# vt-asaplab/vPIN

Measured on AMD Instinct MI355X. Metric: R1CS constraints/sec, whole Spartan SNARK (sat proof + SPARK evaluation proof; vPIN point-mult + point-add instances), higher is better.
Workload: dtype u256 (integers mod q and mod p = 2^255-19, 32-bit limbs); 1 GPU; vPIN LeNet trace (layers L1..L7): 12 SNARKs per step; inputs=resident in HBM, parallelism=one trace per rank x 1 rank(s), no collective; 4 stream(s) per rank, table_slot_bytes=128

## Files before the change

vpin_amd/csrc/msm.hip:

```cpp
#include <algorithm>
#include <atomic>
#include <cstdlib>
#include <condition_variable>
#include <cstring>
#include <memory>
#include <mutex>
#include <string>
#include <vector>

#include "ctx.h"
#include "fp_dev.h"
#include "fp10_dev.h"
#include "ge_tree_dev.h"
#include "mailbox_dev.h"

#ifndef VPIN_NIELS_SLOT
#define VPIN_NIELS_SLOT 96
#endif
static_assert(VPIN_NIELS_SLOT == 96 || VPIN_NIELS_SLOT == 128, "table entry size");

struct vpin_gens {
  vpin::fp* table = nullptr;
  vpin::fp* table_hi = nullptr;
  int s32 = VPIN_NIELS_SLOT / 32;
// ... 217 lines not shown
  int off = w * c, word = off >> 5, sh = off & 31;
  uint32_t lo = s.v[word], hi = (word + 1 < 8) ? s.v[word + 1] : 0u;
  uint64_t both = ((uint64_t)hi << 32) | lo;
  return (uint32_t)(both >> sh) & ((1u << c) - 1u);
}

__device__ __forceinline__ uint32_t carry_into(const fq& s, int w0, int c) {
  const uint32_t half = 1u << (c - 1);
  for (int w = w0 - 1; w >= 0; w--) {
    uint32_t d = scalar_digit(s, w, c);
    if (d != half) return d > half ? 1u : 0u;
  }
  return 0u;
}

__device__ __forceinline__ void table_mul_acc_range(ge_ext& acc, const fq& s_in, const TableSeg& sg, int w0, int w1) {
  fq s = s_in;
  const bool flip = fq_fold_sign(s);
  uint32_t carry = carry_into(s, w0, sg.c);
  const uint32_t full = 1u << sg.c, half = 1u << (sg.c - 1);
#pragma unroll 1
  for (int w = w0; w < w1; w++) {
    uint32_t v = scalar_digit(s, w, sg.c) + carry;
    bool neg = v > half;
    uint32_t mag = neg ? full - v : v;
    carry = neg ? 1u : 0u;
    if (mag != 0) acc = ge_add_niels(acc, niels_load(sg.entry(w, mag - 1)), neg != flip);
  }
}


constexpr int kMsmBlock = 256;
constexpr unsigned kSharedPad = 40000u;
constexpr int kSeg = 8192;

template <bool TEN>
__global__ __launch_bounds__(kMsmBlock, 3) void msm_rows_kernel(const fq* __restrict__ Z, size_t stride, size_t ncols,
                                                             const fq* __restrict__ extra, int n_extra, size_t extra_base0,
                                                             TableView tv, ge_ext* __restrict__ out) {
  const size_t row = blockIdx.x;
  RowAcc<TEN> acc;
  const size_t total = ncols + (size_t)n_extra;
  if (ncols >= 256 && (ncols & (ncols - 1)) == 0 && ((size_t)1 << (tv.nbt - tv.sum0 - 1)) >= ncols) {
    const fq* zr = Z + row * stride;
    const fq first = fq_load(zr);
    if (fq_same(first, fq_load(zr + 1)) && fq_same(first, fq_load(zr + ncols / 2)) && fq_same(first, fq_load(zr + ncols - 1))) {
      int same = 1;
      for (size_t j = threadIdx.x; j < ncols; j += kMsmBlock) same &= fq_same(first, fq_load(zr + j)) ? 1 : 0;
      if (__syncthreads_and(same)) {
        if (threadIdx.x == 0) {
          if (blockIdx.y == 0) {
            if (!fq_is_zero(first)) acc.mul_acc(fq_from_mont(first), tv, tv.sum0 + (size_t)(63 - __builtin_clzll((unsigned long long)ncols)));
            for (int e = 0; e < n_extra; e++) {
              const fq x = fq_load(extra + row * (size_t)n_extra + e);
              if (!fq_is_zero(x)) acc.mul_acc(fq_from_mont(x), tv, extra_base0 + e);
            }
          }
          ge_ext* o = out + row * gridDim.y + blockIdx.y;
          const ge_ext av = acc.ext();
          fp_store(&o->X, av.X); fp_store(&o->Y, av.Y); fp_store(&o->Z, av.Z); fp_store(&o->T, av.T);
        }
        return;
      }
    }
  }
  const size_t per = (total + gridDim.y - 1) / gridDim.y;
  const size_t j0 = (size_t)blockIdx.y * per, j1 = (j0 + per < total) ? j0 + per : total;
  __shared__ uint16_t nz_list[kSeg];
  __shared__ uint32_t nz_count;
  for (size_t seg = j0; seg < j1; seg += kSeg) {
    const size_t seg_end = (seg + kSeg < j1) ? seg + kSeg : j1;
    if (threadIdx.x == 0) nz_count = 0;
    __syncthreads();
    for (size_t j = seg + threadIdx.x; j < seg_end; j += kMsmBlock) {
      const fq* sp = (j < ncols) ? (Z + row * stride + j) : (extra + row * (size_t)n_extra + (j - ncols));
      if (!fq_is_zero(fq_load(sp))) nz_list[atomicAdd(&nz_count, 1u)] = (uint16_t)(j - seg);
    }
    __syncthreads();
    const uint32_t cnt = nz_count;
    for (uint32_t k = threadIdx.x; k < cnt; k += kMsmBlock) {
      const size_t j = seg + nz_list[k];
      fq s;
      size_t base;
      if (j < ncols) { s = fq_load(Z + row * stride + j); base = j; }
      else { s = fq_load(extra + row * (size_t)n_extra + (j - ncols)); base = extra_base0 + (j - ncols); }
      acc.mul_acc(fq_from_mont(s), tv, base);
    }
    __syncthreads();
  }
  __shared__ ge_ext sh[kMsmBlock];
  sh[threadIdx.x] = acc.ext();
  __syncthreads();
  ge_tree_quad(sh, kMsmBlock);
  if (threadIdx.x == 0) {
    const ge_ext av = sh[0];
    ge_ext* o = out + row * gridDim.y + blockIdx.y;
    fp_store(&o->X, av.X); fp_store(&o->Y, av.Y); fp_store(&o->Z, av.Z); fp_store(&o->T, av.T);
  }
}

struct HotRows {
  const uint32_t* idx[3];
  uint32_t hot[3];
  const ge_cached* T[3];
  size_t row0, rows_per_vec;
};

__global__ __launch_bounds__(64) void scalar_times_bases_kernel(const fq* __restrict__ vp, size_t n, TableView tv,
                                                                ge_cached* __restrict__ T) {
  const size_t j = (size_t)blockIdx.x * 64 + threadIdx.x;
  if (j >= n) return;
  const fq v = fq_load(vp);
  ge_ext acc = ge_identity();
  if (!fq_is_zero(v)) table_mul_acc(acc, fq_from_mont(v), tv, j);
  const ge_cached cch = ge_to_cached(acc);
  fp_store(&T[j].YpX, cch.YpX); fp_store(&T[j].YmX, cch.YmX); fp_store(&T[j].Z, cch.Z); fp_store(&T[j].T2d, cch.T2d);
}

template <bool TEN>
__global__ __launch_bounds__(kMsmBlock, 3) void msm_rows_hot_kernel(const fq* __restrict__ Z, size_t stride, size_t ncols, TableView tv,
                                                                 HotRows hr, ge_ext* __restrict__ out, size_t row_base, size_t row_step,
                                                                 int z_compact, const uint8_t* __restrict__ strip_flag) {
  const size_t row = row_base + (size_t)blockIdx.x * row_step;
  const fq* zr = Z + (z_compact ? (size_t)blockIdx.x : row) * stride;
  RowAcc<TEN> acc;
  const bool hot_only = strip_flag && strip_flag[blockIdx.x];
  if (!hot_only && ncols >= 256 && (ncols & (ncols - 1)) == 0 && ((size_t)1 << (tv.nbt - tv.sum0 - 1)) >= ncols) {
    const fq first = fq_load(zr);
    if (fq_same(first, fq_load(zr + 1)) && fq_same(first, fq_load(zr + ncols / 2)) && fq_same(first, fq_load(zr + ncols - 1))) {
      int same = 1;
      for (size_t j = threadIdx.x; j < ncols; j += kMsmBlock) same &= fq_same(first, fq_load(zr + j)) ? 1 : 0;
      if (__syncthreads_and(same)) {
        if (threadIdx.x == 0) {
          if (blockIdx.y == 0 && !fq_is_zero(first)) acc.mul_acc(fq_from_mont(first), tv, tv.sum0 + (size_t)(63 - __builtin_clzll((unsigned long long)ncols)));
          ge_ext* o = out + (size_t)blockIdx.x * gridDim.y + blockIdx.y;
          const ge_ext av = acc.ext();
          fp_store(&o->X, av.X); fp_store(&o->Y, av.Y); fp_store(&o->Z, av.Z); fp_store(&o->T, av.T);
        }
        return;
      }
    }
  }
  const uint32_t* idx = nullptr;
  const ge_cached* T = nullptr;
  uint32_t hot = 0xffffffffu;
  if (row >= hr.row0 && row < hr.row0 + 3 * hr.rows_per_vec) {
    const size_t m = (row - hr.row0) / hr.rows_per_vec;
    if (hr.hot[m] != 0xffffffffu) {
      hot = hr.hot[m];
      T = hr.T[m];
      idx = hr.idx[m] + (row - hr.row0 - m * hr.rows_per_vec) * ncols;
    }
  }
  __shared__ uint16_t list[kSeg];
  __shared__ uint32_t n_front, n_back;
  const size_t per = (ncols + gridDim.y - 1) / gridDim.y;
  const size_t c0 = (size_t)blockIdx.y * per, c1 = (c0 + per < ncols) ? c0 + per : ncols;
  for (size_t seg = c0; seg < c1; seg += kSeg) {
    const size_t seg_end = (seg + kSeg < c1) ? seg + kSeg : c1;
    if (threadIdx.x == 0) { n_front = 0; n_back = 0; }
    __syncthreads();
    for (size_t j = seg + threadIdx.x; j < seg_end; j += kMsmBlock) {
      if (fq_is_zero(fq_load(zr + j))) continue;
      if (idx && idx[j] == hot) list[kSeg - 1 - atomicAdd(&n_back, 1u)] = (uint16_t)(j - seg);
      else if (!hot_only) list[atomicAdd(&n_front, 1u)] = (uint16_t)(j - seg);
    }
    __syncthreads();
    const uint32_t nf = n_front, nb = n_back;
    for (uint32_t k = threadIdx.x; k < nf; k += kMsmBlock) {
      const size_t j = seg + list[k];
      acc.mul_acc(fq_from_mont(fq_load(zr + j)), tv, j);
    }
    for (uint32_t k = threadIdx.x; k < nb; k += kMsmBlock) {
      const ge_cached* t = T + seg + list[kSeg - 1 - k];
      ge_cached q;
      q.YpX = fp_load(&t->YpX); q.YmX = fp_load(&t->YmX); q.Z = fp_load(&t->Z); q.T2d = fp_load(&t->T2d);
      acc.add_cached(q);
    }
    __syncthreads();
  }
  __shared__ ge_ext sh[kMsmBlock];
  sh[threadIdx.x] = acc.ext();
  __syncthreads();
  ge_tree_quad(sh, kMsmBlock);
  if (threadIdx.x == 0) {
    const ge_ext av = sh[0];
    ge_ext* o = out + (size_t)blockIdx.x * gridDim.y + blockIdx.y;
    fp_store(&o->X, av.X); fp_store(&o->Y, av.Y); fp_store(&o->Z, av.Z); fp_store(&o->T, av.T);
  }
}



__global__ __launch_bounds__(kMsmBlock) void strip_classify_kernel(const fq* __restrict__ Z, size_t stride, size_t ncols, HotRows hr,
                                                                    size_t row_base, size_t row_step, int z_compact,
                                                                    uint8_t* __restrict__ flag) {
  const size_t row = row_base + (size_t)blockIdx.x * row_step;
  const fq* zr = Z + (z_compact ? (size_t)blockIdx.x : row) * stride;
  const uint32_t* idx = nullptr;
  uint32_t hot = 0xffffffffu;
  if (hr.rows_per_vec && row >= hr.row0 && row < hr.row0 + 3 * hr.rows_per_vec) {
    const size_t m = (row - hr.row0) / hr.rows_per_vec;
    if (hr.hot[m] != 0xffffffffu) { hot = hr.hot[m]; idx = hr.idx[m] + (row - hr.row0 - m * hr.rows_per_vec) * ncols; }
  }
  const fq first = fq_load(zr);
  int same = 1;
  uint32_t skipped = 0;
  for (size_t j = threadIdx.x; j < ncols; j += kMsmBlock) {
    const fq v = fq_load(zr + j);
    same &= fq_same(first, v) ? 1 : 0;
    skipped += (fq_is_zero(v) || (idx && idx[j] == hot)) ? 1u : 0u;
  }
  __shared__ uint32_t sh[kMsmBlock];
  sh[threadIdx.x] = skipped;
  const int all_same = __syncthreads_and(same);
  for (int st = kMsmBlock / 2; st >= 1; st >>= 1) {
    if ((int)threadIdx.x < st) sh[threadIdx.x] += sh[threadIdx.x + st];
    __syncthreads();
  }
  if (threadIdx.x == 0) flag[blockIdx.x] = (!all_same && sh[0] * 8 <= ncols) ? 1 : 0;
}

__global__ __launch_bounds__(1024) void strip_list_kernel(const uint8_t* __restrict__ flag, size_t nrows, uint32_t* __restrict__ list,
                                                           uint32_t* __restrict__ count) {
  __shared__ uint32_t base[1024];
  const size_t per = (nrows + 1023) / 1024, r0 = (size_t)threadIdx.x * per, r1 = r0 + per < nrows ? r0 + per : nrows;
  uint32_t n = 0;
  for (size_t r = r0; r < r1; r++) n += flag[r] ? 1u : 0u;
  base[threadIdx.x] = n;
  __syncthreads();
  if (threadIdx.x == 0) {
    uint32_t run = 0;
    for (int t = 0; t < 1024; t++) { const uint32_t v = base[t]; base[t] = run; run += v; }
    *count = run;
  }
  __syncthreads();
  uint32_t o = base[threadIdx.x];
  for (size_t r = r0; r < r1; r++)
    if (flag[r]) list[o++] = (uint32_t)r;
}

__global__ __launch_bounds__(256) void strip_trim_kernel(const uint32_t* __restrict__ list, uint32_t* __restrict__ count, uint32_t n_use,
                                                          uint32_t n_all, uint8_t* __restrict__ flag) {
  const uint32_t li = n_use + blockIdx.x * 256 + threadIdx.x;
  if (li < n_all) flag[list[li]] = 0;
  if (blockIdx.x == 0 && threadIdx.x == 0) *count = n_use;
}

__global__ __launch_bounds__(kMsmBlock, 3) void msm_strip_kernel(const fq* __restrict__ Z, size_t stride, size_t ncols, TableView tv, HotRows hr,
                                                                  const uint32_t* __restrict__ list, const uint32_t* __restrict__ list_count,
                                                                  int S, size_t row_base, size_t row_step, int z_compact,
                                                                  ge_ext* __restrict__ parts, uint32_t* __restrict__ sync, int lag) {
  const uint32_t n = *list_count;
  const uint32_t s = blockIdx.x % (uint32_t)S, grp = blockIdx.x / (uint32_t)S;
  if (grp * kMsmBlock >= n) return;
  const uint32_t li = grp * kMsmBlock + threadIdx.x;
  const bool live = li < n;
  const uint32_t i = list[live ? li : n - 1];
  const size_t row = row_base + (size_t)i * row_step;
  const fq* zr = Z + (z_compact ? (size_t)i : row) * stride;
  const uint32_t* idx = nullptr;
  uint32_t hot = 0xffffffffu;
  if (hr.rows_per_vec && row >= hr.row0 && row < hr.row0 + 3 * hr.rows_per_vec) {
    const size_t m = (row - hr.row0) / hr.rows_per_vec;
    if (hr.hot[m] != 0xffffffffu) { hot = hr.hot[m]; idx = hr.idx[m] + (row - hr.row0 - m * hr.rows_per_vec) * ncols; }
  }
  const size_t per = (ncols + (size_t)S - 1) / (size_t)S, j0 = (size_t)s * per, j1 = j0 + per < ncols ? j0 + per : ncols;
  ge10 acc = ge10_identity();
  const uint32_t groups = (n + kMsmBlock - 1) / kMsmBlock;
  uint32_t* my_sync = sync ? sync + (size_t)s * (per + 1) : nullptr;
  __shared__ int sh_nosync;
  if (threadIdx.x == 0) sh_nosync = 0;
  __syncthreads();
  for (size_t j = j0; j < j1; j++) {
    if (my_sync && j - j0 >= (size_t)lag) {
      if (threadIdx.x == 0 && !sh_nosync) {
        long spin = 0;
        while (__hip_atomic_load(my_sync + (j - j0 - (size_t)lag), __ATOMIC_RELAXED, __HIP_MEMORY_SCOPE_AGENT) < groups)
          if (++spin > (1L << 16)) { sh_nosync = 1; break; }
      }
      __syncthreads();
    }
    fq v = fq_load(zr + j);
    const bool act = live && !fq_is_zero(v) && !(idx && idx[j] == hot);
    if (__builtin_amdgcn_ballot_w64(act) != 0) {
      fq sc = fq_from_mont(v);
      if (!act) sc = fq_zero();
      table_mul_acc10(acc, sc, tv, j);
    }
    if (my_sync) {
      __syncthreads();
      if (threadIdx.x == 0) __hip_atomic_fetch_add(my_sync + (j - j0), 1u, __ATOMIC_RELAXED, __HIP_MEMORY_SCOPE_AGENT);
    }
  }
  if (live) {
    const ge_ext av = ge10_to_ext(acc);
    ge_ext* o = parts + (size_t)li * (size_t)S + s;
    fp_store(&o->X, av.X); fp_store(&o->Y, av.Y); fp_store(&o->Z, av.Z); fp_store(&o->T, av.T);
  }
}

__global__ __launch_bounds__(64) void strip_combine_kernel(const ge_ext* __restrict__ parts, const uint32_t* __restrict__ list,
                                                            const uint32_t* __restrict__ list_count, int S, ge_ext* __restrict__ out) {
  const uint32_t li = blockIdx.x * 64 + threadIdx.x;
  if (li >= *list_count) return;
  ge_ext* o = out + list[li];
  ge_ext a;
  a.X = fp_load(&o->X); a.Y = fp_load(&o->Y); a.Z = fp_load(&o->Z); a.T = fp_load(&o->T);
  for (int s = 0; s < S; s++) {
    const ge_ext* p = parts + (size_t)li * (size_t)S + s;
    ge_ext q;
    q.X = fp_load(&p->X); q.Y = fp_load(&p->Y); q.Z = fp_load(&p->Z); q.T = fp_load(&p->T);
    a = ge_add(a, q);
  }
  fp_store(&o->X, a.X); fp_store(&o->Y, a.Y); fp_store(&o->Z, a.Z); fp_store(&o->T, a.T);
}

__device__ __forceinline__ uint32_t count_digits(fq s, const TableView& tv, size_t j) {
  (void)fq_fold_sign(s);
  const TableSeg sg = table_seg(tv, j);
  uint32_t carry = 0, n = 0;
  const uint32_t full = 1u << sg.c, half = 1u << (sg.c - 1);
  for (int w = 0; w < sg.W; w++) {
    uint32_t v = scalar_digit(s, w, sg.c) + carry;
    const bool neg = v > half;
    const uint32_t mag = neg ? full - v : v;
    carry = neg ? 1u : 0u;
    n += mag != 0;
  }
  return n;
}
__global__ __launch_bounds__(kMsmBlock) void msm_count_adds_kernel(const fq* __restrict__ Z, size_t stride, size_t ncols,
                                                                   const fq* __restrict__ extra, int n_extra, size_t extra_base0,
                                                                   TableView tv, unsigned long long* __restrict__ count,
                                                                   HotRows hr = HotRows{}, size_t row_base = 0, size_t row_step = 1,
                                                                   int z_compact = 0) {
  const size_t row = row_base + (size_t)blockIdx.x * row_step;
  const fq* zr = Z + (z_compact ? (size_t)blockIdx.x : row) * stride;
  const uint32_t* hidx = nullptr;
  uint32_t hot = 0xffffffffu;
  if (hr.rows_per_vec && row >= hr.row0 && row < hr.row0 + 3 * hr.rows_per_vec) {
    const size_t m = (row - hr.row0) / hr.rows_per_vec;
    if (hr.hot[m] != 0xffffffffu) { hot = hr.hot[m]; hidx = hr.idx[m] + (row - hr.row0 - m * hr.rows_per_vec) * ncols; }
  }
  uint32_t n = 0;
  bool constant = false;
  if (ncols >= 256 && (ncols & (ncols - 1)) == 0 && ((size_t)1 << (tv.nbt - tv.sum0 - 1)) >= ncols) {
    const fq first = fq_load(zr);
    int same = 1;
    for (size_t j = threadIdx.x; j < ncols; j += kMsmBlock) same &= fq_same(first, fq_load(zr + j)) ? 1 : 0;
    constant = __syncthreads_and(same) != 0;
    if (constant && threadIdx.x == 0 && !fq_is_zero(first))
      n += count_digits(fq_from_mont(first), tv, tv.sum0 + (size_t)(63 - __builtin_clzll((unsigned long long)ncols)));
  }
  if (!constant)
    for (size_t j = threadIdx.x; j < ncols; j += kMsmBlock) {
      const fq s = fq_load(zr + j);
      if (!fq_is_zero(s) && !(hidx && hidx[j] == hot)) n += count_digits(fq_from_mont(s), tv, j);
    }
  for (int e = threadIdx.x; e < n_extra; e += kMsmBlock) {
    const fq x = fq_load(extra + row * (size_t)n_extra + e);
    if (!fq_is_zero(x)) n += count_digits(fq_from_mont(x), tv, extra_base0 + e);
  }
  __shared__ uint32_t sh[kMsmBlock];
  sh[threadIdx.x] = n;
  __syncthreads();
  for (int st = kMsmBlock / 2; st >= 1; st >>= 1) {
    if ((int)threadIdx.x < st) sh[threadIdx.x] += sh[threadIdx.x + st];
    __syncthreads();
  }
  if (threadIdx.x == 0 && sh[0]) atomicAdd(count, (unsigned long long)sh[0]);
}

constexpr int kWideScalars = 32;
template <int Q>
__global__ __launch_bounds__(kMsmBlock) void msm_wide_kernel(const fq* __restrict__ S, size_t ncols, TableView tv,
                                                             fp* __restrict__ parts_xyzt) {
  const size_t row = blockIdx.y;
  const int grp = threadIdx.x & 7;
  ge_ext acc = ge_identity();
#pragma unroll 1
  for (int q = 0; q < Q; q++) {
    const size_t j = ((size_t)blockIdx.x * Q + q) * kWideScalars + (threadIdx.x >> 3);
    if (j < ncols) {
      fq s = fq_load(S + row * ncols + j);
      if (!fq_is_zero(s)) {
        const TableSeg sg = table_seg(tv, j);
        const int wpg = (sg.W + 7) / 8;
        int w0 = grp * wpg, w1 = (w0 + wpg < sg.W) ? w0 + wpg : sg.W;
        if (w0 < w1) table_mul_acc_range(acc, fq_from_mont(s), sg, w0, w1);
      }
    }
  }
  __shared__ ge_ext sh[kMsmBlock];
  sh[threadIdx.x] = acc;
  __syncthreads();
  ge_tree_quad(sh, kMsmBlock);
  if (threadIdx.x == 0) {
    acc = sh[0];
    fp* o = parts_xyzt + 4 * (row * gridDim.x + blockIdx.x);
    fp_store(o, fp_freeze(acc.X)); fp_store(o + 1, fp_freeze(acc.Y)); fp_store(o + 2, fp_freeze(acc.Z)); fp_store(o + 3, fp_freeze(acc.T));
  }
}


struct BulletStep {
  const fq* a_prev; const fq* b_prev;
  fq* a_next; fq* b_next;
  fq* sj;
  size_t n, R;
  int fold, finish, nmsm;
  fq u, u_inv;
  fp* parts;
  uint32_t* up;
  uint32_t seq;
};

__global__ __launch_bounds__(kMsmBlock) void bullet_step_kernel(BulletStep a, TableView tv) {
  const size_t n = a.n;
  const int nip = (int)gridDim.x - a.nmsm;
  if ((int)blockIdx.x < nip) {
    const int ib = (int)blockIdx.x;
    const size_t i = (size_t)ib * kMsmBlock + threadIdx.x;
    fq pl = fq_zero(), pr = fq_zero();
    if (a.finish) {
      if (ib == 0 && threadIdx.x == 0) {
        pl = fq_add(fq_mul(fq_load(a.a_prev), a.u), fq_mul(a.u_inv, fq_load(a.a_prev + 1)));
        pr = fq_add(fq_mul(fq_load(a.b_prev), a.u_inv), fq_mul(a.u, fq_load(a.b_prev + 1)));
      }
    } else if (i < n) {
      fq a0, a1, b0, b1;
      if (a.fold) {
        a0 = fq_add(fq_mul(fq_load(a.a_prev + i), a.u), fq_mul(a.u_inv, fq_load(a.a_prev + 2 * n + i)));
        a1 = fq_add(fq_mul(fq_load(a.a_prev + n + i), a.u), fq_mul(a.u_inv, fq_load(a.a_prev + 3 * n + i)));
        b0 = fq_add(fq_mul(fq_load(a.b_prev + i), a.u_inv), fq_mul(a.u, fq_load(a.b_prev + 2 * n + i)));
        b1 = fq_add(fq_mul(fq_load(a.b_prev + n + i), a.u_inv), fq_mul(a.u, fq_load(a.b_prev + 3 * n + i)));
      } else {
        a0 = fq_load(a.a_prev + i); a1 = fq_load(a.a_prev + n + i);
        b0 = fq_load(a.b_prev + i); b1 = fq_load(a.b_prev + n + i);
      }
      fq_store(a.a_next + i, a0); fq_store(a.a_next + n + i, a1);
      fq_store(a.b_next + i, b0); fq_store(a.b_next + n + i, b1);
      pl = fq_mul(a0, b1);
      pr = fq_mul(a1, b0);
    }
    __shared__ fq shp[kMsmBlock / 64][2];
    const int lane = threadIdx.x & 63, wave = threadIdx.x >> 6;
    pl = fq_wave_sum(pl);
    pr = fq_wave_sum(pr);
    if (lane == 0) { shp[wave][0] = pl; shp[wave][1] = pr; }
    __syncthreads();
    if (threadIdx.x < 2) {
      fq t = shp[0][threadIdx.x];
#pragma unroll
      for (int w = 1; w < kMsmBlock / 64; w++) t = fq_add(t, shp[w][threadIdx.x]);
      publish_scalar(a.up + (2 * (size_t)ib + threadIdx.x) * 12, t, a.seq);
    }
    return;
// ... 468 lines not shown

static int msm_rows_pip(vpin_ctx* c, const vpin_gens* g, const fq* dZ, size_t rows, size_t stride, size_t ncols, const fq* d_extra,
                        int n_extra, size_t extra_base0, int cbits, ge_ext* d_points) {
  DevBuf dgn(c);
  if (dgn.alloc((ncols + 1) * sizeof(ge_niels))) return VPIN_ENOMEM;
  hipLaunchKernelGGL(pip_gens_kernel, dim3((unsigned)((ncols + 1 + 255) / 256)), dim3(256), 0, c->stream, view(g), ncols, extra_base0,
                     n_extra, (ge_niels*)dgn.p);
  return pip_rows(c, (const ge_niels*)dgn.p, dZ, rows, stride, ncols, d_extra, n_extra, cbits, d_points,
                  c->prof_count_adds ? c->d_add_count : nullptr);
}

static int msm_rows(vpin_ctx* c, const vpin_gens* g, const fq* dZ, size_t rows, size_t stride, size_t ncols,
                    const fq* d_extra, int n_extra, size_t extra_base0, ge_ext* d_points) {
  if (const int pm = pip_mode())
    if (n_extra <= 1 && ncols + (size_t)n_extra <= 32768)
      return msm_rows_pip(c, g, dZ, rows, stride, ncols, d_extra, n_extra, extra_base0, pm < 0 ? 0 : pm, d_points);
  double nz_est = (double)rows * ((double)ncols + n_extra);
  size_t total = ncols + (size_t)n_extra;
  int chunks = 1;
  if (rows < 128) {
    size_t want = (total + kMsmBlock - 1) / kMsmBlock * 4;
    chunks = (int)(want < 1 ? 1 : want > 64 ? 64 : want);
  } else if (rows >= 768 && total > (size_t)kSeg) {
    static const int env_chunks = [] { const char* e = getenv("VPIN_MSM_ROW_CHUNKS"); return e ? atoi(e) : 0; }();
    chunks = env_chunks > 0 ? env_chunks : (int)std::min<size_t>(8, (total + kSeg - 1) / kSeg);
  } else if (rows < 768 && total >= 2 * (size_t)kMsmBlock) {
    size_t want = (768 + rows - 1) / rows, most = total / kMsmBlock;
    chunks = (int)(want < most ? want : most);
    if (chunks < 1) chunks = 1;
  }
  DevBuf parts(c);
  ge_ext* dst = d_points;
  if (chunks > 1) {
    if (parts.alloc(rows * (size_t)chunks * sizeof(ge_ext))) return VPIN_ENOMEM;
    dst = (ge_ext*)parts.p;
  }
  if (c->prof_count_adds && c->d_add_count && rows >= 128)
    hipLaunchKernelGGL(msm_count_adds_kernel, dim3((unsigned)rows), dim3(kMsmBlock), 0, c->stream, dZ, stride, ncols, d_extra,
                       n_extra, extra_base0, view(g), c->d_add_count);
  {
    ProfScope ps(c, VPIN_K_MSM, 32.0 * nz_est, rows >= 128 ? VPIN_K_MSM_ROWS : -1);
    static const int env_pad = [] { const char* e = getenv("VPIN_MSM_LDS_PAD"); return e ? atoi(e) : -1; }();
    const unsigned pad = env_pad >= 0 ? (unsigned)env_pad : (c->shared_device ? kSharedPad : 0u);
    if (msm_ten_limbs())
      hipLaunchKernelGGL(msm_rows_kernel<true>, dim3((unsigned)rows, (unsigned)chunks), dim3(kMsmBlock), pad, c->stream, dZ, stride,
                         ncols, d_extra, n_extra, extra_base0, view(g), dst);
    else
      hipLaunchKernelGGL(msm_rows_kernel<false>, dim3((unsigned)rows, (unsigned)chunks), dim3(kMsmBlock), pad, c->stream, dZ, stride,
                         ncols, d_extra, n_extra, extra_base0, view(g), dst);
  }
  if (chunks > 1)
    hipLaunchKernelGGL(ge_sum_chunks_kernel, dim3((unsigned)((rows + 63) / 64)), dim3(64), 0, c->stream, (const ge_ext*)dst,
                       rows, chunks, d_points);
  VPIN_HIP_TRY(hipGetLastError());
  return VPIN_OK;
}

int vpin_hyrax_commit(vpin_ctx* c, const vpin_gens* g, const vpin_table* Z, const uint8_t* blinds, size_t L,
                      size_t blind_base, uint8_t* out_compressed) {
  if (!c || !g || !Z || !Z->d || !blinds || !out_compressed || L == 0) return VPIN_EINVAL;
  if (Z->len % L != 0) return VPIN_ESHAPE;
  size_t R = Z->len / L;
  if (R > g->nb || blind_base >= g->nb) return VPIN_ESHAPE;
  (void)hipSetDevice(c->device);
  DevBuf dbl(c), dpts(c), dout(c);
  if (dbl.alloc(L * 32) || dpts.alloc(L * sizeof(ge_ext)) || dout.alloc(L * 32)) return VPIN_ENOMEM;
  VPIN_HIP_TRY(hipMemcpyAsync(dbl.p, blinds, L * 32, hipMemcpyHostToDevice, c->stream));
  int rc = msm_rows(c, g, Z->d, L, R, R, (const fq*)dbl.p, 1, blind_base, (ge_ext*)dpts.p);
  if (rc) return rc;
  hipLaunchKernelGGL(ge_compress_kernel, dim3((unsigned)((L + 63) / 64)), dim3(64), 0, c->stream, (const ge_ext*)dpts.p, L,
                     (fp*)dout.p, (fp*)nullptr);
  VPIN_HIP_TRY(hipGetLastError());
  VPIN_HIP_TRY(hipMemcpyAsync(out_compressed, dout.p, L * 32, hipMemcpyDeviceToHost, c->stream));
  VPIN_HIP_TRY(hipStreamSynchronize(c->stream));
  return VPIN_OK;
}


int vpin_hyrax_commit_pippenger(vpin_ctx* c, const vpin_gens* g, const vpin_table* Z, const uint8_t* blinds, size_t L,
                                size_t blind_base, int c_bits, uint8_t* out_compressed) {
  if (!c || !g || !Z || !Z->d || !out_compressed || L == 0) return VPIN_EINVAL;
  if (Z->len % L != 0) return VPIN_ESHAPE;
  const size_t R = Z->len / L;
  if (R > g->nb || (blinds && blind_base >= g->nb)) return VPIN_ESHAPE;
  (void)hipSetDevice(c->device);
  const int n_extra = blinds ? 1 : 0;
  DevBuf dbl(c), dpts(c), dout(c);
  if (dbl.alloc(L * 32) || dpts.alloc(L * sizeof(ge_ext)) || dout.alloc(L * 32)) return VPIN_ENOMEM;
  if (blinds) VPIN_HIP_TRY(hipMemcpyAsync(dbl.p, blinds, L * 32, hipMemcpyHostToDevice, c->stream));
  int rc = msm_rows_pip(c, g, Z->d, L, R, R, (const fq*)dbl.p, n_extra, blind_base, c_bits, (ge_ext*)dpts.p);
  if (rc) return rc;
  hipLaunchKernelGGL(ge_compress_kernel, dim3((unsigned)((L + 63) / 64)), dim3(64), 0, c->stream, (const ge_ext*)dpts.p, L,
                     (fp*)dout.p, (fp*)nullptr);
  VPIN_HIP_TRY(hipGetLastError());
  VPIN_HIP_TRY(hipMemcpyAsync(out_compressed, dout.p, L * 32, hipMemcpyDeviceToHost, c->stream));
  VPIN_HIP_TRY(hipStreamSynchronize(c->stream));
  return VPIN_OK;
}

}

namespace vpin {

int hyrax_commit_derefs_hot(vpin_ctx* c, const vpin_gens* g, const vpin_table* Z, size_t L, size_t N, const uint32_t* const col_idx[3],
                            const uint32_t hot[3], const fq* e_ry, uint8_t* out_compressed, size_t row0, size_t nrows, size_t row_step,
                            const fq* z_rows) {
  if (!c || !g || !Z || (!Z->d && !z_rows) || !col_idx || !hot || !e_ry || !out_compressed || L == 0 || Z->len % L) return VPIN_EINVAL;
  const size_t R = Z->len / L;
  if (R > g->nb || N % R || Z->len < 6 * N) return VPIN_ESHAPE;
  const fq* zbase = z_rows ? z_rows : (const fq*)Z->d;
  const int z_compact = z_rows ? 1 : 0;
  if (nrows == (size_t)-1) { row0 = 0; nrows = L; row_step = 1; }
  if (row_step == 0 || (nrows && row0 + (nrows - 1) * row_step >= L)) return VPIN_ESHAPE;
  if (nrows == 0) return VPIN_OK;
  if (pip_mode()) return hyrax_commit_rows_strided(c, g, Z, L, row0, nrows, row_step, out_compressed, z_rows);
  (void)hipSetDevice(c->device);
  DevBuf dpts(c), dout(c), dT(c);
  if (dpts.alloc(nrows * sizeof(ge_ext)) || dout.alloc(nrows * 32)) return VPIN_ENOMEM;
  HotRows hr{};
  hr.row0 = 3 * (N / R);
  hr.rows_per_vec = N / R;
  uint32_t distinct[3];
  int nd = 0;
  for (int m = 0; m < 3; m++) {
    hr.idx[m] = col_idx[m];
    hr.hot[m] = hot[m];
    if (hot[m] == 0xffffffffu) continue;
    bool seen = false;
    for (int k = 0; k < nd; k++) seen = seen || distinct[k] == hot[m];
    if (!seen) distinct[nd++] = hot[m];
  }
  if (nd && dT.alloc((size_t)nd * R * sizeof(ge_cached))) return VPIN_ENOMEM;
  for (int k = 0; k < nd; k++) {
    ge_cached* Tk = (ge_cached*)dT.p + (size_t)k * R;
    hipLaunchKernelGGL(scalar_times_bases_kernel, dim3((unsigned)((R + 63) / 64)), dim3(64), 0, c->stream, e_ry + distinct[k], R, view(g), Tk);
    for (int m = 0; m < 3; m++)
      if (hot[m] == distinct[k]) hr.T[m] = Tk;
  }
  if (c->prof_count_adds && c->d_add_count)
    hipLaunchKernelGGL(msm_count_adds_kernel, dim3((unsigned)nrows), dim3(kMsmBlock), 0, c->stream, zbase, R, R, (const fq*)nullptr, 0,
                       (size_t)0, view(g), c->d_add_count, hr, row0, row_step, z_compact);
  static const int env_chunks = [] { const char* e = getenv("VPIN_MSM_HOT_CHUNKS"); return e ? atoi(e) : 0; }();
  const int chunks = env_chunks > 0 ? env_chunks : (int)std::max<size_t>(1, std::min<size_t>(8, R / kSeg));
  DevBuf dparts(c);
  if (chunks > 1 && dparts.alloc(nrows * (size_t)chunks * sizeof(ge_ext))) return VPIN_ENOMEM;
  const char* es = getenv("VPIN_MSM_STRIP");
  const char* em = getenv("VPIN_MSM_STRIP_MIN");
  const int env_strip = es ? atoi(es) : -1;
  const size_t min_rows = em ? (size_t)atol(em) : 8192, min_list = em ? (size_t)1 : 4096, min_R = em ? (size_t)64 : 4096;
  int S = env_strip > 0 ? env_strip : 16;
  DevBuf dflag(c), dlist(c), dsparts(c), dsync(c);
  uint32_t n_strip = 0;
  bool uniform_shape = false;
  const bool strip_shared = getenv("VPIN_MSM_STRIP_SHARED") != nullptr;
  if (env_strip != 0 && (env_strip > 0 || ((!c->shared_device || strip_shared) && c->comm == nullptr)) && msm_ten_limbs() && nrows >= min_rows && R >= min_R && R <= g->split &&
      S % 8 == 0 && (size_t)S <= R / 8) {
    if (dflag.alloc(nrows) || dlist.alloc((nrows + 1) * sizeof(uint32_t))) return VPIN_ENOMEM;
    uint32_t* d_list = (uint32_t*)dlist.p;
    uint32_t* d_count = d_list + nrows;
    hipLaunchKernelGGL(strip_classify_kernel, dim3((unsigned)nrows), dim3(kMsmBlock), 0, c->stream, zbase, R, R, hr, row0, row_step, z_compact,
                       (uint8_t*)dflag.p);
    hipLaunchKernelGGL(strip_list_kernel, dim3(1), dim3(1024), 0, c->stream, (const uint8_t*)dflag.p, nrows, d_list, d_count);
    VPIN_HIP_TRY(hipMemcpyAsync(&n_strip, d_count, sizeof n_strip, hipMemcpyDeviceToHost, c->stream));
    VPIN_HIP_TRY(hipStreamSynchronize(c->stream));
    if (n_strip < min_list) n_strip = 0;
    if (n_strip && env_strip < 0) {
      const uint32_t found = n_strip;
      const size_t slots = (size_t)c->num_cus * (c->shared_device ? 1 : 3), G = ((size_t)n_strip + kMsmBlock - 1) / kMsmBlock;
      size_t bestG = 0;
      int bestS = 0;
      for (int cand = 8; cand <= 64 && (size_t)cand * 128 <= R; cand += 8)
        if (G * (size_t)cand <= slots) { bestG = G; bestS = cand; }
      if (c->cu_masked)
        for (int cand = 8; cand <= 64 && (size_t)cand * 128 <= R; cand += 8) {
          const size_t g2 = std::min(G, slots / (size_t)cand);
          if (g2 * kMsmBlock >= min_list && g2 * (size_t)cand > bestG * (size_t)bestS) { bestG = g2; bestS = cand; }
        }
      if (const char* eshape = getenv("VPIN_MSM_STRIP_SHAPE")) {
        int eg = 0, esn = 0;
        if (sscanf(eshape, "%d,%d", &eg, &esn) == 2 && eg > 0 && esn > 0 && esn % 8 == 0 && (size_t)esn <= R / 8) {
          if (std::min(G, (size_t)eg) * (size_t)esn <= slots) { bestG = std::min(G, (size_t)eg); bestS = esn; }
          else if (getenv("VPIN_MSM_STRIP_TRACE")) fprintf(stderr, "[strip] VPIN_MSM_STRIP_SHAPE=%d,%d refused: %zu workgroups on %zu slots\n", eg, esn, std::min(G, (size_t)eg) * (size_t)esn, slots);
        }
      }
      const uint32_t n_use = bestG ? (uint32_t)std::min<size_t>(n_strip, bestG * kMsmBlock) : 0;
      if (n_use == 0) {
        n_strip = 0;
      } else {
        if (n_use < n_strip)
          hipLaunchKernelGGL(strip_trim_kernel, dim3((n_strip - n_use + 255) / 256), dim3(256), 0, c->stream, (const uint32_t*)d_list, d_count,
                             n_use, n_strip, (uint8_t*)dflag.p);
        n_strip = n_use;
        S = bestS;
        uniform_shape = true;
      }
      if (getenv("VPIN_MSM_STRIP_TRACE")) fprintf(stderr, "[strip] %zu rows: %u eligible, %u taken as %zu groups x %d strips on %zu slots\n", nrows, found, n_use, bestG, bestS, slots);
    }
    if (n_strip && dsparts.alloc((size_t)n_strip * (size_t)S * sizeof(ge_ext))) return VPIN_ENOMEM;
  }
  const uint8_t* d_flag = n_strip ? (const uint8_t*)dflag.p : nullptr;
  {
    ProfScope ps(c, VPIN_K_MSM, 32.0 * (double)(nrows * R), VPIN_K_MSM_ROWS);
    static const int env_pad = [] { const char* e = getenv("VPIN_MSM_LDS_PAD"); return e ? atoi(e) : -1; }();
    const unsigned pad = env_pad >= 0 ? (unsigned)env_pad : (c->shared_device ? kSharedPad : 0u);
    if (n_strip) {
      c->strip_rows_taken += n_strip;
      const unsigned groups = (unsigned)((n_strip + kMsmBlock - 1) / kMsmBlock);
      const size_t per = (R + (size_t)S - 1) / (size_t)S;
      const char* el = getenv("VPIN_MSM_STRIP_LAG");
      const int lag = el ? atoi(el) : 1;
      uint32_t* d_sync = nullptr;
      if (lag > 0 && uniform_shape) {
        if (dsync.alloc((size_t)S * (per + 1) * sizeof(uint32_t))) return VPIN_ENOMEM;
        d_sync = (uint32_t*)dsync.p;
        VPIN_HIP_TRY(hipMemsetAsync(d_sync, 0, (size_t)S * (per + 1) * sizeof(uint32_t), c->stream));
      }
      hipLaunchKernelGGL(msm_strip_kernel, dim3(groups * (unsigned)S), dim3(kMsmBlock), pad, c->stream, zbase, R, R, view(g), hr,
                         (const uint32_t*)dlist.p, (const uint32_t*)dlist.p + nrows, S, row0, row_step, z_compact, (ge_ext*)dsparts.p,
                         d_sync, lag);
    }
    if (msm_ten_limbs())
      hipLaunchKernelGGL(msm_rows_hot_kernel<true>, dim3((unsigned)nrows, (unsigned)chunks), dim3(kMsmBlock), pad, c->stream, zbase,
                         R, R, view(g), hr, chunks > 1 ? (ge_ext*)dparts.p : (ge_ext*)dpts.p, row0, row_step, z_compact, d_flag);
    else
      hipLaunchKernelGGL(msm_rows_hot_kernel<false>, dim3((unsigned)nrows, (unsigned)chunks), dim3(kMsmBlock), pad, c->stream, zbase,
                         R, R, view(g), hr, chunks > 1 ? (ge_ext*)dparts.p : (ge_ext*)dpts.p, row0, row_step, z_compact, d_flag);
    if (chunks > 1)
      hipLaunchKernelGGL(ge_sum_chunks_kernel, dim3((unsigned)((nrows + 63) / 64)), dim3(64), 0, c->stream, (const ge_ext*)dparts.p, nrows,
                         chunks, (ge_ext*)dpts.p);
    if (n_strip)
      hipLaunchKernelGGL(strip_combine_kernel, dim3((n_strip + 63) / 64), dim3(64), 0, c->stream, (const ge_ext*)dsparts.p,
                         (const uint32_t*)dlist.p, (const uint32_t*)dlist.p + nrows, S, (ge_ext*)dpts.p);
  }
  hipLaunchKernelGGL(ge_compress_kernel, dim3((unsigned)((nrows + 63) / 64)), dim3(64), 0, c->stream, (const ge_ext*)dpts.p, nrows,
                     (fp*)dout.p, (fp*)nullptr);
  VPIN_HIP_TRY(hipGetLastError());
  VPIN_HIP_TRY(hipMemcpyAsync(out_compressed, dout.p, nrows * 32, hipMemcpyDeviceToHost, c->stream));
  VPIN_HIP_TRY(hipStreamSynchronize(c->stream));
  return VPIN_OK;
}

int hyrax_commit_rows_strided(vpin_ctx* c, const vpin_gens* g, const vpin_table* Z, size_t L, size_t row0, size_t nrows, size_t row_step,
                              uint8_t* out_compressed, const fq* z_rows) {
  if (!c || !g || !Z || (!Z->d && !z_rows) || !out_compressed || L == 0 || row_step == 0) return VPIN_EINVAL;
  if (nrows == 0) return VPIN_OK;
  if (Z->len % L != 0 || row0 + (nrows - 1) * row_step >= L) return VPIN_ESHAPE;
  const size_t R = Z->len / L;
  if (R > g->nb) return VPIN_ESHAPE;
  (void)hipSetDevice(c->device);
  DevBuf dpts(c), dout(c);
  if (dpts.alloc(nrows * sizeof(ge_ext)) || dout.alloc(nrows * 32)) return VPIN_ENOMEM;
  int rc = z_rows ? msm_rows(c, g, z_rows, nrows, R, R, nullptr, 0, 0, (ge_ext*)dpts.p)
                  : msm_rows(c, g, Z->d + row0 * R, nrows, row_step * R, R, nullptr, 0, 0, (ge_ext*)dpts.p);
  if (rc) return rc;
  hipLaunchKernelGGL(ge_compress_kernel, dim3((unsigned)((nrows + 63) / 64)), dim3(64), 0, c->stream, (const ge_ext*)dpts.p, nrows,
                     (fp*)dout.p, (fp*)nullptr);
  VPIN_HIP_TRY(hipGetLastError());
  VPIN_HIP_TRY(hipMemcpyAsync(out_compressed, dout.p, nrows * 32, hipMemcpyDeviceToHost, c->stream));
  VPIN_HIP_TRY(hipStreamSynchronize(c->stream));
  return VPIN_OK;
}

}

extern "C" {

int vpin_hyrax_commit_rows(vpin_ctx* c, const vpin_gens* g, const vpin_table* Z, size_t L, size_t row0, size_t nrows,
                           const uint8_t* blinds, size_t blind_base, uint8_t* out_compressed) {
  if (!c || !g || !Z || !Z->d || !out_compressed || L == 0 || nrows == 0) return VPIN_EINVAL;
  if (Z->len % L != 0 || row0 + nrows > L) return VPIN_ESHAPE;
  const size_t R = Z->len / L;
  if (R > g->nb || (blinds && blind_base >= g->nb)) return VPIN_ESHAPE;
  (void)hipSetDevice(c->device);
  DevBuf dbl(c), dpts(c), dout(c);
  if ((blinds && dbl.alloc(nrows * 32)) || dpts.alloc(nrows * sizeof(ge_ext)) || dout.alloc(nrows * 32)) return VPIN_ENOMEM;
  if (blinds) VPIN_HIP_TRY(hipMemcpyAsync(dbl.p, blinds, nrows * 32, hipMemcpyHostToDevice, c->stream));
  int rc = msm_rows(c, g, Z->d + row0 * R, nrows, R, R, blinds ? (const fq*)dbl.p : nullptr, blinds ? 1 : 0, blind_base, (ge_ext*)dpts.p);
  if (rc) return rc;
  hipLaunchKernelGGL(ge_compress_kernel, dim3((unsigned)((nrows + 63) / 64)), dim3(64), 0, c->stream, (const ge_ext*)dpts.p, nrows,
                     (fp*)dout.p, (fp*)nullptr);
  VPIN_HIP_TRY(hipGetLastError());
  VPIN_HIP_TRY(hipMemcpyAsync(out_compressed, dout.p, nrows * 32, hipMemcpyDeviceToHost, c->stream));
  VPIN_HIP_TRY(hipStreamSynchronize(c->stream));
  return VPIN_OK;
}

int vpin_hyrax_commit_pair(vpin_ctx* c, const vpin_gens* g, const vpin_table* Za, const vpin_table* Zb,
                           const uint8_t* blinds_a, const uint8_t* blinds_b, size_t L, size_t blind_base,
                           uint8_t* out_a, uint8_t* out_b, uint8_t* out_sum) {
  if (!c || !g || !Za || !Zb || !blinds_a || !blinds_b || !out_a || !out_b || !out_sum || L == 0) return VPIN_EINVAL;
  if (Za->len != Zb->len || Za->len % L != 0) return VPIN_ESHAPE;
  size_t R = Za->len / L;
  if (R > g->nb || blind_base >= g->nb) return VPIN_ESHAPE;
  (void)hipSetDevice(c->device);
  DevBuf dbl(c), dpts(c), dout(c);
  if (dbl.alloc(2 * L * 32) || dpts.alloc(3 * L * sizeof(ge_ext)) || dout.alloc(3 * L * 32)) return VPIN_ENOMEM;
  VPIN_HIP_TRY(hipMemcpyAsync(dbl.p, blinds_a, L * 32, hipMemcpyHostToDevice, c->stream));
  VPIN_HIP_TRY(hipMemcpyAsync((uint8_t*)dbl.p + L * 32, blinds_b, L * 32, hipMemcpyHostToDevice, c->stream));
  ge_ext* pts = (ge_ext*)dpts.p;
  int rc = msm_rows(c, g, Za->d, L, R, R, (const fq*)dbl.p, 1, blind_base, pts);
  if (rc) return rc;
  rc = msm_rows(c, g, Zb->d, L, R, R, (const fq*)dbl.p + L, 1, blind_base, pts + L);
  if (rc) return rc;
  hipLaunchKernelGGL(ge_add_rows_kernel, dim3((unsigned)((L + 63) / 64)), dim3(64), 0, c->stream, pts, pts + L, L, pts + 2 * L);
  hipLaunchKernelGGL(ge_compress_kernel, dim3((unsigned)((3 * L + 63) / 64)), dim3(64), 0, c->stream, (const ge_ext*)pts, 3 * L,
                     (fp*)dout.p, (fp*)nullptr);
  VPIN_HIP_TRY(hipGetLastError());
  VPIN_HIP_TRY(hipMemcpyAsync(out_a, dout.p, L * 32, hipMemcpyDeviceToHost, c->stream));
  VPIN_HIP_TRY(hipMemcpyAsync(out_b, (uint8_t*)dout.p + L * 32, L * 32, hipMemcpyDeviceToHost, c->stream));
  VPIN_HIP_TRY(hipMemcpyAsync(out_sum, (uint8_t*)dout.p + 2 * L * 32, L * 32, hipMemcpyDeviceToHost, c->stream));
  VPIN_HIP_TRY(hipStreamSynchronize(c->stream));
  return VPIN_OK;
}

constexpr size_t kMaxParts = 128;
static inline int wide_q(size_t ncols) { return ncols >= 8192 ? 4 : 1; }
static inline size_t raw_parts(size_t ncols) { const size_t per = (size_t)kWideScalars * wide_q(ncols); return (ncols + per - 1) / per; }
size_t vpin_gens_msm_parts_count(size_t ncols) { size_t n = raw_parts(ncols); return n < kMaxParts ? n : kMaxParts; }

int vpin_gens_msm_parts(vpin_ctx* c, const vpin_gens* g, const uint8_t* scalars_mont, size_t rows, size_t ncols,
                        uint8_t* parts_xyzt) {
  if (!c || !g || !scalars_mont || !parts_xyzt || rows == 0 || ncols == 0) return VPIN_EINVAL;
  if (ncols > g->nb) return VPIN_ESHAPE;
  (void)hipSetDevice(c->device);
  DevBuf ds(c);
  if (ds.alloc(rows * ncols * 32)) return VPIN_ENOMEM;
  VPIN_HIP_TRY(hipMemcpyAsync(ds.p, scalars_mont, rows * ncols * 32, hipMemcpyHostToDevice, c->stream));
  return vpin::gens_msm_parts_dev(c, g, (const fq*)ds.p, rows, ncols, parts_xyzt);
}

}

namespace vpin {
struct CommitPairState {
  DevBuf pts;
  size_t L = 0;
  explicit CommitPairState(vpin_ctx* c) : pts(c) {}
};

int commit_pair_begin(vpin_ctx* c, const vpin_gens* g, const vpin_table* Za, const vpin_table* Zb, size_t L_all,
                      CommitPairState** out, size_t row0, size_t nrows, size_t row_step) {
  if (!c || !g || !Za || !Zb || !out || L_all == 0) return VPIN_EINVAL;
  if (Za->len != Zb->len || Za->len % L_all != 0) return VPIN_ESHAPE;
  size_t R = Za->len / L_all;
  if (R > g->nb) return VPIN_ESHAPE;
  if (nrows == (size_t)-1) { row0 = 0; nrows = L_all; row_step = 1; }
  if (nrows == 0 || row_step == 0 || row0 + (nrows - 1) * row_step >= L_all) return VPIN_ESHAPE;
  const size_t L = nrows;
  (void)hipSetDevice(c->device);
  CommitPairState* st = new (std::nothrow) CommitPairState(c);
  if (!st) return VPIN_ENOMEM;
  st->L = L;
  if (st->pts.alloc(5 * L * sizeof(ge_ext))) { delete st; return VPIN_ENOMEM; }
  ge_ext* pts = (ge_ext*)st->pts.p;
  int rc = msm_rows(c, g, Za->d + row0 * R, L, row_step * R, R, nullptr, 0, 0, pts);
  if (!rc) rc = msm_rows(c, g, Zb->d + row0 * R, L, row_step * R, R, nullptr, 0, 0, pts + L);
  if (rc) { delete st; return rc; }
  *out = st;
  return VPIN_OK;
}

int commit_pair_finish(vpin_ctx* c, const vpin_gens* g, CommitPairState* st, const uint8_t* blinds_a, const uint8_t* blinds_b,
                       size_t blind_base, uint8_t* out_a, uint8_t* out_b, uint8_t* out_sum) {
  if (!st) return VPIN_EINVAL;
  std::unique_ptr<CommitPairState> guard(st);
  if (!c || !g || !blinds_a || !blinds_b || !out_a || !out_b || !out_sum) return VPIN_EINVAL;
  if (blind_base >= g->nb) return VPIN_ESHAPE;
  const size_t L = st->L;
  DevBuf dbl(c), dout(c);
  if (dbl.alloc(2 * L * 32) || dout.alloc(3 * L * 32)) return VPIN_ENOMEM;
  VPIN_HIP_TRY(hipMemcpyAsync(dbl.p, blinds_a, L * 32, hipMemcpyHostToDevice, c->stream));
  VPIN_HIP_TRY(hipMemcpyAsync((uint8_t*)dbl.p + L * 32, blinds_b, L * 32, hipMemcpyHostToDevice, c->stream));
  ge_ext* pts = (ge_ext*)st->pts.p;
  hipLaunchKernelGGL(single_base_mul_kernel, dim3((unsigned)((2 * L + 7) / 8)), dim3(64), 0, c->stream, (const fq*)dbl.p, 2 * L,
                     view(g), blind_base, pts + 2 * L);
  const unsigned gb = (unsigned)((2 * L + 63) / 64);
  hipLaunchKernelGGL(ge_add_rows_kernel, dim3(gb), dim3(64), 0, c->stream, pts, pts + 2 * L, 2 * L, pts + 2 * L);
  hipLaunchKernelGGL(ge_add_rows_kernel, dim3((unsigned)((L + 63) / 64)), dim3(64), 0, c->stream, pts + 2 * L, pts + 3 * L, L,
                     pts + 4 * L);
  hipLaunchKernelGGL(ge_compress_kernel, dim3((unsigned)((3 * L + 63) / 64)), dim3(64), 0, c->stream,
                     (const ge_ext*)(pts + 2 * L), 3 * L, (fp*)dout.p, (fp*)nullptr);
  VPIN_HIP_TRY(hipGetLastError());
  VPIN_HIP_TRY(hipMemcpyAsync(out_a, dout.p, L * 32, hipMemcpyDeviceToHost, c->stream));
  VPIN_HIP_TRY(hipMemcpyAsync(out_b, (uint8_t*)dout.p + L * 32, L * 32, hipMemcpyDeviceToHost, c->stream));
  VPIN_HIP_TRY(hipMemcpyAsync(out_sum, (uint8_t*)dout.p + 2 * L * 32, L * 32, hipMemcpyDeviceToHost, c->stream));
// ... 120 lines not shown
```

Measured before the change: 72.91 million constraints/s.

## Split strip MSM into multiple passes and early-exit cold rows in hot-only kernel

Lets the strip-parallel MSM path cover rows beyond the first launch's capacity by issuing several strip passes, each with its own group count and strip width, and its own parts and sync sub-buffers. It also passes the strip row count as a kernel argument instead of reading it from device memory, and makes hot-only row blocks with no hot index write the identity and return immediately. Extra passes are off by default (VPIN_MSM_STRIP_PASSES defaults to 1), so by default only the early exit and the argument change apply. The cost is more launches and more bookkeeping when multiple passes are enabled.

```diff
diff --git a/vpin_amd/csrc/msm.hip b/vpin_amd/csrc/msm.hip
--- a/vpin_amd/csrc/msm.hip
+++ b/vpin_amd/csrc/msm.hip
@@ -393,6 +393,14 @@
       idx = hr.idx[m] + (row - hr.row0 - m * hr.rows_per_vec) * ncols;
     }
   }
+  if (hot_only && !idx) {
+    if (threadIdx.x == 0) {
+      ge_ext* o = out + (size_t)blockIdx.x * gridDim.y + blockIdx.y;
+      const ge_ext av = acc.ext();
+      fp_store(&o->X, av.X); fp_store(&o->Y, av.Y); fp_store(&o->Z, av.Z); fp_store(&o->T, av.T);
+    }
+    return;
+  }
   __shared__ uint16_t list[kSeg];
   __shared__ uint32_t n_front, n_back;
   const size_t per = (ncols + gridDim.y - 1) / gridDim.y;
@@ -402,6 +410,10 @@
     if (threadIdx.x == 0) { n_front = 0; n_back = 0; }
     __syncthreads();
     for (size_t j = seg + threadIdx.x; j < seg_end; j += kMsmBlock) {
+      if (hot_only) {
+        if (idx[j] == hot && !fq_is_zero(fq_load(zr + j))) list[kSeg - 1 - atomicAdd(&n_back, 1u)] = (uint16_t)(j - seg);
+        continue;
+      }
       if (fq_is_zero(fq_load(zr + j))) continue;
       if (idx && idx[j] == hot) list[kSeg - 1 - atomicAdd(&n_back, 1u)] = (uint16_t)(j - seg);
       else if (!hot_only) list[atomicAdd(&n_front, 1u)] = (uint16_t)(j - seg);
@@ -489,10 +501,9 @@
 }
 
 __global__ __launch_bounds__(kMsmBlock, 3) void msm_strip_kernel(const fq* __restrict__ Z, size_t stride, size_t ncols, TableView tv, HotRows hr,
-                                                                  const uint32_t* __restrict__ list, const uint32_t* __restrict__ list_count,
+                                                                  const uint32_t* __restrict__ list, uint32_t n,
                                                                   int S, size_t row_base, size_t row_step, int z_compact,
                                                                   ge_ext* __restrict__ parts, uint32_t* __restrict__ sync, int lag) {
-  const uint32_t n = *list_count;
   const uint32_t s = blockIdx.x % (uint32_t)S, grp = blockIdx.x / (uint32_t)S;
   if (grp * kMsmBlock >= n) return;
   const uint32_t li = grp * kMsmBlock + threadIdx.x;
@@ -542,9 +553,9 @@
 }
 
 __global__ __launch_bounds__(64) void strip_combine_kernel(const ge_ext* __restrict__ parts, const uint32_t* __restrict__ list,
-                                                            const uint32_t* __restrict__ list_count, int S, ge_ext* __restrict__ out) {
+                                                            uint32_t n, int S, ge_ext* __restrict__ out) {
   const uint32_t li = blockIdx.x * 64 + threadIdx.x;
-  if (li >= *list_count) return;
+  if (li >= n) return;
   ge_ext* o = out + list[li];
   ge_ext a;
   a.X = fp_load(&o->X); a.Y = fp_load(&o->Y); a.Z = fp_load(&o->Z); a.T = fp_load(&o->T);
@@ -1319,6 +1330,13 @@
   DevBuf dflag(c), dlist(c), dsparts(c), dsync(c);
   uint32_t n_strip = 0;
   bool uniform_shape = false;
+  struct StripPass { uint32_t off, n; int S; };
+  constexpr int kMaxStripPasses = 8;
+  StripPass pass[kMaxStripPasses];
+  int npass = 0;
+  const char* ep = getenv("VPIN_MSM_STRIP_PASSES");
+  const int max_passes = std::max(1, std::min(kMaxStripPasses, ep ? atoi(ep) : 1));
+  const bool strip_trace = getenv("VPIN_MSM_STRIP_TRACE") != nullptr;
   const bool strip_shared = getenv("VPIN_MSM_STRIP_SHARED") != nullptr;
   if (env_strip != 0 && (env_strip > 0 || ((!c->shared_device || strip_shared) && c->comm == nullptr)) && msm_ten_limbs() && nrows >= min_rows && R >= min_R && R <= g->split &&
       S % 8 == 0 && (size_t)S <= R / 8) {
@@ -1343,27 +1361,55 @@
           const size_t g2 = std::min(G, slots / (size_t)cand);
           if (g2 * kMsmBlock >= min_list && g2 * (size_t)cand > bestG * (size_t)bestS) { bestG = g2; bestS = cand; }
         }
+      bool forced = false;
       if (const char* eshape = getenv("VPIN_MSM_STRIP_SHAPE")) {
         int eg = 0, esn = 0;
         if (sscanf(eshape, "%d,%d", &eg, &esn) == 2 && eg > 0 && esn > 0 && esn % 8 == 0 && (size_t)esn <= R / 8) {
-          if (std::min(G, (size_t)eg) * (size_t)esn <= slots) { bestG = std::min(G, (size_t)eg); bestS = esn; }
-          else if (getenv("VPIN_MSM_STRIP_TRACE")) fprintf(stderr, "[strip] VPIN_MSM_STRIP_SHAPE=%d,%d refused: %zu workgroups on %zu slots\n", eg, esn, std::min(G, (size_t)eg) * (size_t)esn, slots);
+          if (std::min(G, (size_t)eg) * (size_t)esn <= slots) { bestG = std::min(G, (size_t)eg); bestS = esn; forced = true; }
+          else if (strip_trace) fprintf(stderr, "[strip] VPIN_MSM_STRIP_SHAPE=%d,%d refused: %zu workgroups on %zu slots\n", eg, esn, std::min(G, (size_t)eg) * (size_t)esn, slots);
         }
       }
-      const uint32_t n_use = bestG ? (uint32_t)std::min<size_t>(n_strip, bestG * kMsmBlock) : 0;
-      if (n_use == 0) {
+      uint32_t taken = 0;
+      if (bestG) {
+        pass[npass++] = StripPass{0, (uint32_t)std::min<size_t>(n_strip, bestG * kMsmBlock), bestS};
+        taken = pass[0].n;
+      }
+      while (taken && taken < n_strip && npass < max_passes) {
+        const size_t left = ((size_t)(n_strip - taken) + kMsmBlock - 1) / kMsmBlock;
+        size_t pg = forced ? std::min(left, bestG) : 0;
+        int ps = forced ? bestS : 0;
+        if (!forced)
+          for (int cand = 8; cand <= 128 && (size_t)cand * 128 <= R; cand += 8) {
+            const size_t g2 = std::min(left, slots / (size_t)cand);
+            if (g2 * (size_t)cand > pg * (size_t)ps) { pg = g2; ps = cand; }
+          }
+        if (pg == 0) break;
+        pass[npass] = StripPass{taken, (uint32_t)std::min<size_t>(n_strip - taken, pg * kMsmBlock), ps};
+        taken += pass[npass++].n;
+      }
+      if (taken == 0) {
         n_strip = 0;
       } else {
-        if (n_use < n_strip)
-          hipLaunchKernelGGL(strip_trim_kernel, dim3((n_strip - n_use + 255) / 256), dim3(256), 0, c->stream, (const uint32_t*)d_list, d_count,
-                             n_use, n_strip, (uint8_t*)dflag.p);
-        n_strip = n_use;
-        S = bestS;
+        if (taken < n_strip)
+          hipLaunchKernelGGL(strip_trim_kernel, dim3((n_strip - taken + 255) / 256), dim3(256), 0, c->stream, (const uint32_t*)d_list, d_count,
+                             taken, n_strip, (uint8_t*)dflag.p);
+        n_strip = taken;
         uniform_shape = true;
       }
-      if (getenv("VPIN_MSM_STRIP_TRACE")) fprintf(stderr, "[strip] %zu rows: %u eligible, %u taken as %zu groups x %d strips on %zu slots\n", nrows, found, n_use, bestG, bestS, slots);
-    }
-    if (n_strip && dsparts.alloc((size_t)n_strip * (size_t)S * sizeof(ge_ext))) return VPIN_ENOMEM;
+      if (strip_trace) {
+        fprintf(stderr, "[strip] %zu rows: %u eligible, %u taken as %zu groups x %d strips on %zu slots", nrows, found, taken, bestG, bestS, slots);
+        for (int p = 1; p < npass; p++) fprintf(stderr, " + %u rows as %u x %d", pass[p].n, (pass[p].n + kMsmBlock - 1) / kMsmBlock, pass[p].S);
+        fprintf(stderr, "\n");
+      }
+    } else if (n_strip) {
+      pass[npass++] = StripPass{0, n_strip, S};
+    }
+    size_t nparts = 0;
+    for (int p = 0; p < npass; p++) nparts += (size_t)pass[p].n * (size_t)pass[p].S;
+    if (n_strip && dsparts.alloc(nparts * sizeof(ge_ext))) return VPIN_ENOMEM;
+  } else if (strip_trace && env_strip != 0) {
+    fprintf(stderr, "[strip] %zu rows of %zu: not taken (shared %d, comm %d, masked %d, num_cus %d)\n", nrows, R, (int)c->shared_device,
+            c->comm != nullptr, (int)c->cu_masked, (int)c->num_cus);
   }
   const uint8_t* d_flag = n_strip ? (const uint8_t*)dflag.p : nullptr;
   {
@@ -1372,19 +1418,25 @@
     const unsigned pad = env_pad >= 0 ? (unsigned)env_pad : (c->shared_device ? kSharedPad : 0u);
     if (n_strip) {
       c->strip_rows_taken += n_strip;
-      const unsigned groups = (unsigned)((n_strip + kMsmBlock - 1) / kMsmBlock);
-      const size_t per = (R + (size_t)S - 1) / (size_t)S;
       const char* el = getenv("VPIN_MSM_STRIP_LAG");
       const int lag = el ? atoi(el) : 1;
+      size_t nsync = 0;
+      for (int p = 0; p < npass; p++) nsync += (size_t)pass[p].S * ((R + (size_t)pass[p].S - 1) / (size_t)pass[p].S + 1);
       uint32_t* d_sync = nullptr;
       if (lag > 0 && uniform_shape) {
-        if (dsync.alloc((size_t)S * (per + 1) * sizeof(uint32_t))) return VPIN_ENOMEM;
+        if (dsync.alloc(nsync * sizeof(uint32_t))) return VPIN_ENOMEM;
         d_sync = (uint32_t*)dsync.p;
-        VPIN_HIP_TRY(hipMemsetAsync(d_sync, 0, (size_t)S * (per + 1) * sizeof(uint32_t), c->stream));
+        VPIN_HIP_TRY(hipMemsetAsync(d_sync, 0, nsync * sizeof(uint32_t), c->stream));
       }
-      hipLaunchKernelGGL(msm_strip_kernel, dim3(groups * (unsigned)S), dim3(kMsmBlock), pad, c->stream, zbase, R, R, view(g), hr,
-                         (const uint32_t*)dlist.p, (const uint32_t*)dlist.p + nrows, S, row0, row_step, z_compact, (ge_ext*)dsparts.p,
-                         d_sync, lag);
+      size_t at_parts = 0, at_sync = 0;
+      for (int p = 0; p < npass; p++) {
+        const unsigned groups = (pass[p].n + kMsmBlock - 1) / kMsmBlock;
+        hipLaunchKernelGGL(msm_strip_kernel, dim3(groups * (unsigned)pass[p].S), dim3(kMsmBlock), pad, c->stream, zbase, R, R, view(g), hr,
+                           (const uint32_t*)dlist.p + pass[p].off, pass[p].n, pass[p].S, row0, row_step, z_compact,
+                           (ge_ext*)dsparts.p + at_parts, d_sync ? d_sync + at_sync : nullptr, lag);
+        at_parts += (size_t)pass[p].n * (size_t)pass[p].S;
+        at_sync += (size_t)pass[p].S * ((R + (size_t)pass[p].S - 1) / (size_t)pass[p].S + 1);
+      }
     }
     if (msm_ten_limbs())
       hipLaunchKernelGGL(msm_rows_hot_kernel<true>, dim3((unsigned)nrows, (unsigned)chunks), dim3(kMsmBlock), pad, c->stream, zbase,
@@ -1395,9 +1447,12 @@
     if (chunks > 1)
       hipLaunchKernelGGL(ge_sum_chunks_kernel, dim3((unsigned)((nrows + 63) / 64)), dim3(64), 0, c->stream, (const ge_ext*)dparts.p, nrows,
                          chunks, (ge_ext*)dpts.p);
-    if (n_strip)
-      hipLaunchKernelGGL(strip_combine_kernel, dim3((n_strip + 63) / 64), dim3(64), 0, c->stream, (const ge_ext*)dsparts.p,
-                         (const uint32_t*)dlist.p, (const uint32_t*)dlist.p + nrows, S, (ge_ext*)dpts.p);
+    size_t at_parts = 0;
+    for (int p = 0; p < (n_strip ? npass : 0); p++) {
+      hipLaunchKernelGGL(strip_combine_kernel, dim3((pass[p].n + 63) / 64), dim3(64), 0, c->stream, (const ge_ext*)dsparts.p + at_parts,
+                         (const uint32_t*)dlist.p + pass[p].off, pass[p].n, pass[p].S, (ge_ext*)dpts.p);
+      at_parts += (size_t)pass[p].n * (size_t)pass[p].S;
+    }
   }
   hipLaunchKernelGGL(ge_compress_kernel, dim3((unsigned)((nrows + 63) / 64)), dim3(64), 0, c->stream, (const ge_ext*)dpts.p, nrows,
                      (fp*)dout.p, (fp*)nullptr);
```

After: 72.82 million constraints/s, median of 6. About the same (-0.1%).
